# lunarring/latentblending

Measured on NVIDIA H100. Metric: transition frames/sec (1024^2 SDXL, 30 steps, 15 branches), higher is better.
Workload: dtype f16

## Files before the change

include/lb200.h:

```cpp
#ifndef LB200_H
#define LB200_H

#include <stddef.h>
#include <stdint.h>

#ifdef __cplusplus
extern "C" {
#endif

#define LB_ABI_VERSION 2

typedef struct lb_ctx lb_ctx;

int         lb_abi_version(void);
const char* lb_last_error(void);
int lb_ctx_create(int device, lb_ctx** out);
int lb_ctx_destroy(lb_ctx* ctx);
int lb_ctx_sm_count(lb_ctx* ctx);

size_t lb_slerp_workspace_bytes(int64_t rows, int64_t n);
int lb_slerp_rows(lb_ctx* ctx, const void* p0_dev, const void* p1_dev, void* out_dev,
                  int64_t rows, int64_t n, int64_t stride0, int64_t stride1, int64_t stride_out,
                  int dtype, double fract, const double* fract_rows_dev,
                  void* workspace_dev, void* stream);
// ... 17 lines not shown
    int32_t taps;
    const void* w; int64_t w_ld;
    int32_t N;
    const void* bias;
    const void* bias2; int64_t bias2_ld;
    const void* res; int64_t res_ld;
    void* out; int64_t out_ld;
    int32_t mode;
    const void* ln_stats; int32_t ln_parts;
    const void* ln_csum; const void* ln_bias;
    float ln_eps;
    void* stats_out; int32_t stats_parts;
} lb_gemm_desc;
#define LB_GEMM_STATIC_W 0x100
#define LB_GEMM_RELU 0x200
#define LB_GEMM_GEGLU256 0x400
int lb_gemm(lb_ctx* ctx, const lb_gemm_desc* desc, void* stream);
int lb_gemm_stats_parts(lb_ctx* ctx, const lb_gemm_desc* desc);

typedef struct lb_attn_desc {
    const void* q; int64_t q_ld; int32_t q_col0;
    const void* k; int64_t k_ld; int32_t k_col0;
    const void* v; int64_t v_ld; int32_t v_col0;
    void* out; int64_t out_ld;
    int32_t B, heads, Sq, Skv, head_dim;
    float scale;
} lb_attn_desc;
int lb_attention(lb_ctx* ctx, const lb_attn_desc* desc, void* stream);

size_t lb_groupnorm_workspace_bytes(lb_ctx* ctx, int B, int HW, int groups);
int lb_groupnorm(lb_ctx* ctx, const void* x, int64_t ld, int B, int HW, int C, int groups,
// ... 82 lines not shown
```

latentblending_b200/_cabi.py:

```python
import ctypes
import os
import threading

_HERE = os.path.dirname(os.path.abspath(__file__))
LIB_PATH = os.path.join(_HERE, "liblb200.so")

c_void_p, c_int, c_int64, c_float, c_double, c_size_t = (
    ctypes.c_void_p, ctypes.c_int, ctypes.c_int64, ctypes.c_float, ctypes.c_double, ctypes.c_size_t)

class GemmDesc(ctypes.Structure):
    _fields_ = [("a0", c_void_p), ("a0_ld", c_int64), ("a0_c", ctypes.c_int32),
                ("a1", c_void_p), ("a1_ld", c_int64), ("a1_c", ctypes.c_int32),
                ("B", ctypes.c_int32), ("H", ctypes.c_int32), ("W", ctypes.c_int32),
                ("taps", ctypes.c_int32),
                ("w", c_void_p), ("w_ld", c_int64),
                ("N", ctypes.c_int32),
                ("bias", c_void_p),
                ("bias2", c_void_p), ("bias2_ld", c_int64),
                ("res", c_void_p), ("res_ld", c_int64),
                ("out", c_void_p), ("out_ld", c_int64),
                ("mode", ctypes.c_int32),
                ("ln_stats", c_void_p), ("ln_parts", ctypes.c_int32),
                ("ln_csum", c_void_p), ("ln_bias", c_void_p), ("ln_eps", c_float),
                ("stats_out", c_void_p), ("stats_parts", ctypes.c_int32)]
# ... 47 lines not shown
    _fields_ = [("x", c_void_p), ("ld_x", c_int64), ("H", c_int32), ("W", c_int32), ("C", c_int32), ("k", c_int32),
                ("stride", c_int32), ("pad", c_int32), ("out", c_void_p), ("ld_out", c_int64), ("f", c_float * 6)]


class _OpUnion(ctypes.Union):
    _fields_ = [("gemm", GemmDesc), ("attn", AttnDesc), ("norm", _NormOp), ("embed", _EmbedOp), ("lin", _LinOp),
                ("conv", _ConvOp), ("resample", _ResampleOp), ("aux", _AuxOp), ("patch", _PatchOp)]


class Op(ctypes.Structure):
    _fields_ = [("kind", c_int32), ("reserved", c_int32), ("u", _OpUnion)]


GEMM_STATIC_W = 0x100
GEMM_RELU = 0x200
GEMM_GEGLU256 = 0x400
(OP_GEMM, OP_ATTENTION, OP_GROUPNORM, OP_LAYERNORM, OP_EMBED_INPUTS, OP_LINEAR_SMALL, OP_CONV_IN, OP_CONV_OUT,
 OP_UPSAMPLE2X, OP_IM2COL_S2, OP_LATENT_PREP, OP_SOFTMAX_ROWS, OP_POSTPROCESS_U8, OP_LPIPS_IM2COL_U8, OP_IM2COL,
 OP_MAXPOOL3S2, OP_NHWC_TO_NCHW) = range(1, 18)


SIGNATURES = {
    "lb_abi_version": (c_int, []),
    "lb_last_error": (ctypes.c_char_p, []),
    "lb_ctx_create": (c_int, [c_int, ctypes.POINTER(c_void_p)]),
    "lb_ctx_destroy": (c_int, [c_void_p]),
    "lb_ctx_sm_count": (c_int, [c_void_p]),
    "lb_slerp_workspace_bytes": (c_size_t, [c_int64, c_int64]),
    "lb_slerp_rows": (c_int, [c_void_p, c_void_p, c_void_p, c_void_p, c_int64, c_int64, c_int64, c_int64, c_int64,
                              c_int, c_double, c_void_p, c_void_p, c_void_p]),
    "lb_lerp": (c_int, [c_void_p, c_void_p, c_void_p, c_void_p, c_int64, c_int, c_double, c_void_p]),
# ... 98 lines not shown
```

latentblending_b200/csrc/gemm_sm90.cu:

```cuda
#include "gemm_sm90.cuh"
#include <stdlib.h>

#include "sm90.cuh"

using namespace sm90;

namespace {

constexpr int kBM = 128;
constexpr int kBK = 64;
constexpr int kEpiParts = 4;
constexpr int kThreadsGemm = 384;
constexpr int kABytes = kBM * kBK * 2;

template <int BN> struct Cfg {
    static constexpr int b_bytes = BN * kBK * 2;
    static constexpr int stage_bytes = kABytes + b_bytes;
    static constexpr int deep = (BN <= 64) ? 8 : (BN <= 128) ? 7 : (BN <= 160) ? 6 : 4;
    static constexpr int smem_bytes(int nst) { return nst * stage_bytes + 1024  + 256 ; }
};

__device__ __forceinline__ float gelu_erf(float x) {
    const float z = fabsf(x) * 0.70710678118654752440f;
    const float t = __frcp_rn(fmaf(0.3275911f, z, 1.0f));
    float poly = fmaf(1.061405429f, t, -1.453152027f);
    poly = fmaf(poly, t, 1.421413741f);
    poly = fmaf(poly, t, -0.284496736f);
    poly = fmaf(poly, t, 0.254829592f);
    const float erfc_abs = poly * t * exp2f(-1.4426950408889634f * z * z);
    const float one_plus_erf = x >= 0.f ? 2.0f - erfc_abs : erfc_abs;
    return 0.5f * x * one_plus_erf;
}

__device__ __forceinline__ float2 ld_h2(const __half* p) {
    return __half22float2(__ldg(reinterpret_cast<const __half2*>(p)));
}
__device__ __forceinline__ float2 ld_f2(const float* p) { return __ldg(reinterpret_cast<const float2*>(p)); }

__device__ __forceinline__ void ln_row_stats(const GemmParams& p, long long row, bool ok, float& mu, float& rstd) {
    mu = 0.f;
    rstd = 1.f;
    if (!ok) return;
    float s = 0.f, q = 0.f;
    const float4* st = reinterpret_cast<const float4*>(p.ln_stats + row * p.ln_parts);
    const int pairs = p.ln_parts >> 1;
    for (int base = 0; base < pairs; base += 8) {
        float4 v[8];
#pragma unroll
        for (int i = 0; i < 8; ++i) v[i] = (base + i < pairs) ? __ldcg(st + base + i) : make_float4(0.f, 0.f, 0.f, 0.f);
#pragma unroll
        for (int i = 0; i < 8; ++i) {
            s += v[i].x;
            q += v[i].y;
            s += v[i].z;
            q += v[i].w;
        }
    }
    mu = s * p.ln_inv_k;
    double var = (double)q * (double)p.ln_inv_k - (double)mu * (double)mu;
    if (var < 0.0) var = 0.0;
    rstd = rsqrtf((float)var + p.ln_eps);
}

template <int BN>
__global__ void __launch_bounds__(kThreadsGemm, 1) gemm_tc_kernel(const __grid_constant__ GemmParams p) {
    using C = Cfg<BN>;
    pdl_launch_dependents();
    extern __shared__ uint8_t smem_raw[];
    const uint32_t raw_addr = smem_u32(smem_raw);
    uint8_t* smem = smem_raw + ((1024u - (raw_addr & 1023u)) & 1023u);
    uint8_t* smem_a = smem;
    const int nst = p.stages;
    uint8_t* smem_b = smem + nst * kABytes;
    uint64_t* bars = reinterpret_cast<uint64_t*>(smem + nst * C::stage_bytes);
    uint64_t* full = bars;
    uint64_t* empty = bars + nst;

    const int warp = uniform_warp_idx(), lane = threadIdx.x & 31;
    const int wg = warp >> 2;

    if (warp == 0 && lane == 0) {
        tma_prefetch_desc(&p.tmA[0]);
        tma_prefetch_desc(&p.tmA[1]);
        tma_prefetch_desc(&p.tmB);
        for (int s = 0; s < nst; ++s) {
            mbar_init(&full[s], 1);
            mbar_init(&empty[s], 2);
        }
        fence_mbar_init();
    }
    __syncthreads();

    const int m_groups = p.tiles_m;
    const int num_tiles = m_groups * p.tiles_n;
    const int tile0 = (int)blockIdx.x;
    const int tile_step = (int)gridDim.x;

    int early_kb = 0;
    if (p.static_w && tile0 < num_tiles) early_kb = p.total_kb < nst ? p.total_kb : nst;
    if (warp == 0 && early_kb > 0) {
        if (elect_one()) {
            const int n_tile = tile0 / m_groups;
            for (int kb = 0; kb < early_kb; ++kb) {
// ... 30 lines not shown
                            tma_load_2d(smem_b + stage * C::b_bytes, &p.tmB, &full[stage], kb_global * kBK, n_tile * BN);
                        }
                    }
                    __syncwarp();
                    if (++stage == nst) { stage = 0; phase ^= 1; }
                }
            }
        }
        return;
    }

    reg_alloc<232>();
    const int cw = wg - 1;
    const bool wg_leader = (threadIdx.x & 127) == 0;
    const int quad = lane & 3;
    int rr[2], ww[2], hh[2], bb[2];
#pragma unroll
    for (int i = 0; i < 2; ++i) {
        rr[i] = cw * 64 + (warp & 3) * 16 + (lane >> 2) + 8 * i;
        ww[i] = rr[i] % p.tw;
        hh[i] = (rr[i] / p.tw) % p.th;
        bb[i] = rr[i] / (p.tw * p.th);
    }
    float acc[BN / 2];
    int stage = 0;
    uint32_t phase = 0;
    for (int tile = tile0; tile < num_tiles; tile += tile_step) {
        const int m_tile = tile % m_groups, n_tile = tile / m_groups;
        bool row_ok[2];
        long long row[2];
        int bidx[2];
        float ln_mu[2] = {0.f, 0.f}, ln_rstd[2] = {1.f, 1.f};
#pragma unroll
        for (int i = 0; i < 2; ++i) {
            const int x = (m_tile % p.tiles_x) * p.tw + ww[i];
            const int y = ((m_tile / p.tiles_x) % p.tiles_y) * p.th + hh[i];
            const int b = (m_tile / (p.tiles_x * p.tiles_y)) * p.tb + bb[i];
            row_ok[i] = (x < p.W) && (y < p.H) && (b < p.B);
            row[i] = ((long long)b * p.H + y) * p.W + x;
            bidx[i] = b;
            if (p.ln_stats) ln_row_stats(p, row[i], row_ok[i], ln_mu[i], ln_rstd[i]);
        }
        int prev_stage = -1;
        for (int kb = 0; kb < p.total_kb; ++kb) {
            mbar_wait(&full[stage], phase, p.err_flag, 3);
            const uint32_t a_addr = smem_u32(smem_a + stage * kABytes) + cw * (64 * 128);
            const uint32_t b_addr = smem_u32(smem_b + stage * C::b_bytes);
            fence_regs(acc);
            wgmma_fence();
#pragma unroll
            for (int k = 0; k < kBK / 16; ++k)
                WgmmaSS<BN>::template mma<0>(acc, make_smem_desc_sw128(a_addr + k * 32, 16, 1024),
                                             make_smem_desc_sw128(b_addr + k * 32, 16, 1024), (kb | k) != 0);
            wgmma_commit();
            wgmma_wait<1>();
            fence_regs(acc);
            if (prev_stage >= 0 && wg_leader) mbar_arrive(&empty[prev_stage]);
            prev_stage = stage;
            if (++stage == nst) { stage = 0; phase ^= 1; }
        }
        wgmma_wait<0>();
        fence_regs(acc);
        if (prev_stage >= 0 && wg_leader) mbar_arrive(&empty[prev_stage]);

        if (p.mode == 0) {
            const int n_base = n_tile * BN + 2 * quad;
#pragma unroll
            for (int i = 0; i < 2; ++i) {
                float st_sum = 0.f, st_sq = 0.f;
                if (row_ok[i]) {
                    const __half* res_row = p.res ? p.res + row[i] * p.ldr : nullptr;
                    __half* out_row = p.out + row[i] * p.ldo;
#pragma unroll
                    for (int j = 0; j < BN / 8; ++j) {
                        const int n = n_base + 8 * j;
                        if (n < p.N) {
                            float v0 = acc[4 * j + 2 * i], v1 = acc[4 * j + 2 * i + 1];
                            if (p.ln_stats) {
                                const float2 c = ld_f2(p.ln_csum + n), t = ld_f2(p.ln_bias + n);
                                v0 = fmaf(ln_rstd[i], v0 - ln_mu[i] * c.x, t.x);
                                v1 = fmaf(ln_rstd[i], v1 - ln_mu[i] * c.y, t.y);
                            } else if (p.bias) {
                                const float2 t = ld_h2(p.bias + n);
                                v0 += t.x;
                                v1 += t.y;
                            }
                            if (p.bias2) {
                                const float2 t = ld_h2(p.bias2 + (long long)bidx[i] * p.bias2_ld + n);
                                v0 += t.x;
                                v1 += t.y;
                            }
                            if (res_row) {
                                const float2 t = __half22float2(*reinterpret_cast<const __half2*>(res_row + n));
                                v0 += t.x;
                                v1 += t.y;
                            }
                            if (p.relu) {
                                v0 = fmaxf(v0, 0.f);
                                v1 = fmaxf(v1, 0.f);
                            }
                            const __half2 o = __floats2half2_rn(v0, v1);
                            *reinterpret_cast<__half2*>(out_row + n) = o;
                            if (p.stats_out) {
                                const float2 f = __half22float2(o);
                                st_sum += f.x + f.y;
                                st_sq = fmaf(f.x, f.x, fmaf(f.y, f.y, st_sq));
                            }
                        }
                    }
                    if (p.stats_out)
                        p.stats_out[row[i] * (kEpiParts * p.tiles_n) + kEpiParts * n_tile + quad] =
                            make_float2(st_sum, st_sq);
                }
            }
        } else {
            constexpr int HN = BN / 2;
            const int o_base = n_tile * HN + 2 * quad;
            const int a_base = n_tile * BN + 2 * quad;
#pragma unroll
            for (int i = 0; i < 2; ++i) {
                if (!row_ok[i]) continue;
                __half* out_row = p.out + row[i] * p.ldo;
#pragma unroll
                for (int j = 0; j < HN / 8; ++j) {
                    float v[2] = {acc[4 * j + 2 * i], acc[4 * j + 2 * i + 1]};
                    float g[2] = {acc[4 * (j + HN / 8) + 2 * i], acc[4 * (j + HN / 8) + 2 * i + 1]};
                    float2 bv = make_float2(0.f, 0.f), bg = make_float2(0.f, 0.f);
                    if (p.ln_stats) {
                        const float2 cv = ld_f2(p.ln_csum + a_base + 8 * j), cg = ld_f2(p.ln_csum + a_base + HN + 8 * j);
                        bv = ld_f2(p.ln_bias + a_base + 8 * j);
                        bg = ld_f2(p.ln_bias + a_base + HN + 8 * j);
                        v[0] = ln_rstd[i] * (v[0] - ln_mu[i] * cv.x);
                        v[1] = ln_rstd[i] * (v[1] - ln_mu[i] * cv.y);
                        g[0] = ln_rstd[i] * (g[0] - ln_mu[i] * cg.x);
                        g[1] = ln_rstd[i] * (g[1] - ln_mu[i] * cg.y);
                    } else if (p.bias) {
                        bv = ld_h2(p.bias + a_base + 8 * j);
                        bg = ld_h2(p.bias + a_base + HN + 8 * j);
                    }
                    const float r0 = lb_round_h(v[0] + bv.x) * lb_round_h(gelu_erf(lb_round_h(g[0] + bg.x)));
                    const float r1 = lb_round_h(v[1] + bv.y) * lb_round_h(gelu_erf(lb_round_h(g[1] + bg.y)));
                    *reinterpret_cast<__half2*>(out_row + o_base + 8 * j) = __floats2half2_rn(r0, r1);
                }
            }
        }
    }
}


typedef CUresult (*EncodeTiledFn)(CUtensorMap*, CUtensorMapDataType, cuuint32_t, void*, const cuuint64_t*,
                                  const cuuint64_t*, const cuuint32_t*, const cuuint32_t*, CUtensorMapInterleave,
                                  CUtensorMapSwizzle, CUtensorMapL2promotion, CUtensorMapFloatOOBfill);

int get_encode(lb_ctx* ctx, EncodeTiledFn* fn) {
    if (!ctx->tmap_encode) {
        void* f = nullptr;
        cudaDriverEntryPointQueryResult qres;
        LB_CHECK_CUDA(cudaGetDriverEntryPoint("cuTensorMapEncodeTiled", &f, cudaEnableDefault, &qres));
        LB_REQUIRE(f != nullptr && qres == cudaDriverEntryPointSuccess, "cuTensorMapEncodeTiled not available");
// ... 32 lines not shown
    cuuint32_t estr[2] = {1, 1};
    CUresult r = enc(m, CU_TENSOR_MAP_DATA_TYPE_FLOAT16, 2, const_cast<void*>(base), dims, strides, box, estr,
                     CU_TENSOR_MAP_INTERLEAVE_NONE, CU_TENSOR_MAP_SWIZZLE_128B, CU_TENSOR_MAP_L2_PROMOTION_L2_256B,
                     CU_TENSOR_MAP_FLOAT_OOB_FILL_NONE);
    LB_REQUIRE(r == CUDA_SUCCESS, "cuTensorMapEncodeTiled(weight K=%lld N=%d bn=%d) failed: %d", (long long)K, N, bn,
               (int)r);
    return 0;
}

bool is_pow2(int v) { return v > 0 && (v & (v - 1)) == 0; }

template <int BN> int launch_bn(const GemmPlan& plan, cudaStream_t st) {
    static bool attr_set = false;
    if (!attr_set) {
        LB_CHECK_CUDA(cudaFuncSetAttribute(gemm_tc_kernel<BN>, cudaFuncAttributeMaxDynamicSharedMemorySize,
                                           Cfg<BN>::smem_bytes(Cfg<BN>::deep)));
        attr_set = true;
    }
    LB_CHECK_CUDA(lb_launch_pdl(gemm_tc_kernel<BN>, dim3((unsigned)plan.grid), dim3(kThreadsGemm),
                                (size_t)Cfg<BN>::smem_bytes(plan.p.stages), st, plan.p));
    return 0;
}

}

int gemm_plan_build(lb_ctx* ctx, const GemmDesc& d, GemmPlan* plan) {
    LB_REQUIRE(ctx && plan, "gemm: null ctx/plan");
    LB_REQUIRE(d.a0 && d.w && d.out, "gemm: null a0/w/out");
    LB_REQUIRE(d.B >= 1 && d.H >= 1 && d.W >= 1 && d.N >= 8, "gemm: bad shape B=%d H=%d W=%d N=%d", d.B, d.H, d.W, d.N);
    LB_REQUIRE(d.taps == 1 || d.taps == 9, "gemm: taps must be 1 or 9");
    LB_REQUIRE(d.a0_c % kBK == 0 && d.a0_c > 0, "gemm: a0 channels (%d) must be a multiple of 64", d.a0_c);
    LB_REQUIRE(d.a1 == nullptr || (d.a1_c % kBK == 0 && d.a1_c > 0), "gemm: a1 channels must be a multiple of 64");
    LB_REQUIRE(d.N % 8 == 0, "gemm: N (%d) must be a multiple of 8", d.N);
    LB_REQUIRE(d.out_ld % 8 == 0 && lb_aligned16(d.out), "gemm: out must be 16B aligned with ld %% 8 == 0");
    LB_REQUIRE(!d.res || (d.res_ld % 8 == 0 && lb_aligned16(d.res)), "gemm: residual alignment");
// ... 10 lines not shown
        th = kBM / tw;
        if (th > d.H) {
            LB_REQUIRE(is_pow2(d.H), "gemm: H (%d) must be a power of two when H*W < 128", d.H);
            th = d.H;
        }
        tb = kBM / (tw * th);
    }
    p.tw = tw; p.th = th; p.tb = tb;
    p.W = d.W; p.H = d.H; p.B = d.B;
    p.tiles_x = (int)lb_ceil_div(d.W, tw);
    p.tiles_y = (int)lb_ceil_div(d.H, th);
    const int tiles_b = (int)lb_ceil_div(d.B, tb);
    p.tiles_m = p.tiles_x * p.tiles_y * tiles_b;
    int bn;
    if ((d.mode & 0xff) == 1) {
        bn = (d.mode & LB_GEMM_GEGLU256) ? 256 : 128;
        LB_REQUIRE(d.N % bn == 0, "gemm: GEGLU needs N %% %d == 0 (got %d)", bn, d.N);
    } else if (d.N % 256 == 0 && (int64_t)p.tiles_m * (d.N / 256) >= 2 * ctx->sm_count) bn = 256;
    else if (d.N % 160 == 0) bn = 160;
    else if (d.N % 128 == 0) bn = 128;
    else if (d.N <= 64) bn = 64;
    else bn = 128;
    plan->bn = bn;
    p.tiles_n = (int)lb_ceil_div(d.N, bn);
    p.N = d.N;
    p.mode = d.mode & 0xff;
    p.static_w = (d.mode & LB_GEMM_STATIC_W) ? 1 : 0;
    int ns = 0, total = 0;
    if (d.taps == 9) {
        for (int ky = 0; ky < 3; ++ky)
            for (int kx = 0; kx < 3; ++kx) {
                p.seg_map[ns] = 0; p.seg_dy[ns] = ky - 1; p.seg_dx[ns] = kx - 1; p.seg_kb[ns] = d.a0_c / kBK;
                total += p.seg_kb[ns++];
            }
    } else {
        p.seg_map[ns] = 0; p.seg_dy[ns] = 0; p.seg_dx[ns] = 0; p.seg_kb[ns] = d.a0_c / kBK;
        total += p.seg_kb[ns++];
    }
    if (d.a1) {
        p.seg_map[ns] = 1; p.seg_dy[ns] = 0; p.seg_dx[ns] = 0; p.seg_kb[ns] = d.a1_c / kBK;
// ... 30 lines not shown
        p.ln_csum = static_cast<const float*>(d.ln_csum);
        p.ln_bias = static_cast<const float*>(d.ln_bias);
        p.ln_inv_k = 1.0f / (float)d.a0_c;
        p.ln_eps = d.ln_eps;
    }
    if (d.stats_out) {
        LB_REQUIRE(p.mode == 0, "gemm: stats_out needs the linear epilogue");
        LB_REQUIRE(d.stats_parts == kEpiParts * p.tiles_n, "gemm: stats_parts must be %d * ceil(N / %d) = %d (got %d)",
                   kEpiParts, bn, kEpiParts * p.tiles_n, d.stats_parts);
        p.stats_out = static_cast<float2*>(d.stats_out);
    }
    {
        const int tiles = p.tiles_m * p.tiles_n;
        plan->grid = tiles < ctx->sm_count ? tiles : ctx->sm_count;
    }
    p.stages = (bn <= 64) ? 8 : (bn <= 128) ? 7 : (bn <= 160) ? 6 : 4;
    return 0;
}

int gemm_plan_launch(const GemmPlan& plan, cudaStream_t st) {
    switch (plan.bn) {
        case 64: return launch_bn<64>(plan, st);
        case 128: return launch_bn<128>(plan, st);
        case 160: return launch_bn<160>(plan, st);
        case 256: return launch_bn<256>(plan, st);
    }
    lb_set_error("gemm: unsupported N tile %d", plan.bn);
    return 2;
}

extern "C" int lb_gemm_stats_parts(lb_ctx* ctx, const lb_gemm_desc* desc) {
// ... 16 lines not shown
```

latentblending_b200/csrc/gemm_sm90.cuh:

```cuda
#pragma once
#include "common.cuh"

struct GemmDesc {
    const void* a0; int64_t a0_ld; int32_t a0_c;
    const void* a1; int64_t a1_ld; int32_t a1_c;
    int32_t B, H, W;
    int32_t taps;
    const void* w; int64_t w_ld;
    int32_t N;
    const void* bias;
    const void* bias2; int64_t bias2_ld;
    const void* res; int64_t res_ld;
    void* out; int64_t out_ld;
    int32_t mode;
    const void* ln_stats; int32_t ln_parts;
    const void* ln_csum; const void* ln_bias; float ln_eps;
    void* stats_out; int32_t stats_parts;
};

constexpr int kGemmMaxSegs = 12;

struct alignas(64) GemmParams {
    CUtensorMap tmA[2];
    CUtensorMap tmB;
    int num_segs;
    int seg_map[kGemmMaxSegs], seg_dy[kGemmMaxSegs], seg_dx[kGemmMaxSegs], seg_kb[kGemmMaxSegs];
    int total_kb;
    int W, H, B;
    int tw, th, tb;
    int tiles_x, tiles_y, tiles_m, tiles_n;
    int N;
    int mode;
    int stages;
    int static_w;
    __half* out; long long ldo;
    const __half* bias;
    const __half* bias2; long long bias2_ld;
    const __half* res; long long ldr;
    int* err_flag;
    int relu;
    const float2* ln_stats; int ln_parts; float ln_inv_k, ln_eps;
    const float* ln_csum; const float* ln_bias;
    float2* stats_out;
};

struct GemmPlan {
    GemmParams p;
    int bn;
// ... 7 lines not shown
```

latentblending_b200/unet.py:

```python
import ctypes
import os
from dataclasses import dataclass
from typing import Tuple

import torch

from . import _cabi
from ._cabi import (GEMM_GEGLU256, GEMM_RELU, GEMM_STATIC_W, OP_ATTENTION, OP_CONV_IN, OP_CONV_OUT, OP_EMBED_INPUTS, OP_GEMM,
                    OP_GROUPNORM, OP_IM2COL, OP_IM2COL_S2, OP_LATENT_PREP, OP_LAYERNORM, OP_LINEAR_SMALL,
                    OP_LPIPS_IM2COL_U8, OP_MAXPOOL3S2, OP_NHWC_TO_NCHW, OP_POSTPROCESS_U8, OP_SOFTMAX_ROWS, OP_UPSAMPLE2X, Op, check, ctx,
                    stream_ptr)


@dataclass
class UNetConfig:
    in_channels: int = 4
    out_channels: int = 4
    block_out_channels: Tuple[int, ...] = (320, 640, 1280)
    layers_per_block: int = 2
    transformer_layers: Tuple[int, ...] = (0, 2, 10)
    head_dim: int = 64
    cross_attention_dim: int = 2048
    addition_time_embed_dim: int = 256
    pooled_dim: int = 1280
# ... 229 lines not shown
    wf = (w.float() * gamma.float()[None, :]).half().contiguous()
    csum = wf.float().sum(dim=1).contiguous()
    lnb = w.float() @ beta.float()
    if bias is not None:
        lnb = lnb + bias.float()
    return wf, csum, lnb.contiguous()


def _geglu_perm(inner, device, half=64):
    idx = torch.arange(inner, device=device).view(-1, half)
    return torch.stack([idx, idx + inner], dim=1).reshape(-1)


class PackedUNet:

    def __init__(self, cfg: UNetConfig, state_dict, device, fold_ln=True, geglu_tile=128):
        self.cfg = cfg
        self.device = torch.device(device)
        self.fold_ln = fold_ln
        self.geglu_tile = geglu_tile
        sd = state_dict
        dev = self.device

        def g(name):
            return sd[name].detach().to(device=dev, dtype=torch.float16).contiguous()

        def conv3(name):
            w = g(name + ".weight")
            return w.permute(0, 2, 3, 1).reshape(w.shape[0], -1).contiguous()

        self.g = g
        self.w = {}
        W = self.w
        W["conv_in.w"] = g("conv_in.weight").permute(2, 3, 1, 0).contiguous()
        W["conv_in.b"] = g("conv_in.bias")
# ... 31 lines not shown
            W[a + ".norm.g"], W[a + ".norm.b"] = g(a + ".norm.weight"), g(a + ".norm.bias")
            W[a + ".proj_in.w"], W[a + ".proj_in.b"] = g(a + ".proj_in.weight"), g(a + ".proj_in.bias")
            W[a + ".proj_out.w"], W[a + ".proj_out.b"] = g(a + ".proj_out.weight"), g(a + ".proj_out.bias")
            depth = 0
            while f"{a}.transformer_blocks.{depth}.norm1.weight" in sd:
                t = f"{a}.transformer_blocks.{depth}"
                for n in ("norm1", "norm2", "norm3"):
                    W[f"{t}.{n}.g"], W[f"{t}.{n}.b"] = g(f"{t}.{n}.weight"), g(f"{t}.{n}.bias")
                wqkv = torch.cat([g(t + ".attn1.to_q.weight"), g(t + ".attn1.to_k.weight"),
                                  g(t + ".attn1.to_v.weight")], 0).contiguous()
                W[t + ".attn1.out.w"], W[t + ".attn1.out.b"] = g(t + ".attn1.to_out.0.weight"), g(t + ".attn1.to_out.0.bias")
                wq = g(t + ".attn2.to_q.weight")
                W[t + ".attn2.kv.w"] = torch.cat([g(t + ".attn2.to_k.weight"), g(t + ".attn2.to_v.weight")], 0).contiguous()
                W[t + ".attn2.out.w"], W[t + ".attn2.out.b"] = g(t + ".attn2.to_out.0.weight"), g(t + ".attn2.to_out.0.bias")
                pw, pb = g(t + ".ff.net.0.proj.weight"), g(t + ".ff.net.0.proj.bias")
                perm = _geglu_perm(pw.shape[0] // 2, dev, half=geglu_tile // 2)
                if fold_ln:
                    for key, w_, b_, nrm, pm in ((".attn1.qkv", wqkv, None, "norm1", None), (".attn2.q", wq, None, "norm2", None),
                                                 (".ff.in", pw, pb, "norm3", perm)):
                        wf, cs, lb = _fold_layernorm(w_, b_, W[f"{t}.{nrm}.g"], W[f"{t}.{nrm}.b"])
                        if pm is not None:
                            wf, cs, lb = wf[pm].contiguous(), cs[pm].contiguous(), lb[pm].contiguous()
                        W[t + key + ".w"], W[t + key + ".csum"], W[t + key + ".lnb"] = wf, cs, lb
                else:
                    W[t + ".attn1.qkv.w"], W[t + ".attn2.q.w"] = wqkv, wq
                    W[t + ".ff.in.w"], W[t + ".ff.in.b"] = pw[perm].contiguous(), pb[perm].contiguous()
                W[t + ".ff.out.w"], W[t + ".ff.out.b"] = g(t + ".ff.net.2.weight"), g(t + ".ff.net.2.bias")
                depth += 1
            W[a + ".depth"] = depth
        for k in sd:
            if k.endswith("samplers.0.conv.weight"):
# ... 2 lines not shown

    def nbytes(self):
        return sum(t.numel() * t.element_size() for t in self.w.values() if torch.is_tensor(t))


class UNetB200:

    def __init__(self, cfg: UNetConfig, state_dict, device="cuda:0", fold_ln=None):
        import os
        self.cfg = cfg
        self.device = torch.device(device)
        self.dev_index = self.device.index or 0
        if fold_ln is None:
            fold_ln = os.environ.get("LB_LN_FOLD") is not None
        self.fold_ln = fold_ln
        tile = int(os.environ.get("LB_GEGLU_TILE", "256"))
        widths = [c for c, d in zip(cfg.block_out_channels, cfg.transformer_layers) if d]
        if tile == 256 and any((8 * c) % 256 for c in widths):
            tile = 128
        self.geglu_tile = tile
        self.packed = PackedUNet(cfg, state_dict, self.device, fold_ln=fold_ln, geglu_tile=tile)
        self._plans = {}

    def plan(self, B, H, W, tag=None, x_in=None):
        key = (B, H, W) if tag is None else (B, H, W, tag)
        if key not in self._plans:
            self._plans[key] = _Lowering(self, B, H, W, x_in=x_in)
        return self._plans[key]

    @torch.no_grad()
    def forward(self, x, t, encoder_hidden_states, text_embeds, time_ids, ctx_changed=True):
        B, _, H, W = x.shape
        pl = self.plan(B, H, W)
        pl.x_in.copy_(x)
        pl.text.copy_(text_embeds)
        pl.tids.copy_(time_ids)
# ... 92 lines not shown
            M = rows_at(level)
            n1 = scratch("n1", M, cin)
            P.groupnorm(x, B, h_ * w_, cin, groups, Wt[rname + ".norm1.g"], Wt[rname + ".norm1.b"], 1e-5, 1, n1, self.ws)
            h1 = scratch("h1", M, cout)
            P.gemm(n1, Wt[rname + ".conv1.w"], cout, B, h_, w_, h1, taps=9, bias=Wt[rname + ".conv1.b"], bias2=tslice(rname))
            n2 = scratch("n2", M, cout)
            P.groupnorm(h1, B, h_ * w_, cout, groups, Wt[rname + ".norm2.g"], Wt[rname + ".norm2.b"], 1e-5, 1, n2, self.ws)
            if Wt.get(rname + ".has_shortcut"):
                P.gemm(n2, Wt[rname + ".conv2.w"], cout, B, h_, w_, out, taps=9, a1=x, a1_c=cin, bias=Wt[rname + ".conv2.b"])
            else:
                P.gemm(n2, Wt[rname + ".conv2.w"], cout, B, h_, w_, out, taps=9, bias=Wt[rname + ".conv2.b"], res=x)

        kv_cache = {}

        fold = net.fold_ln
        geglu_mode = 1 | (GEMM_GEGLU256 if net.geglu_tile == 256 else 0)
        f32 = dict(dtype=torch.float32, device=dev)

        def transformer(aname, x, C, level, out):
            h_, w_ = res_hw[level]
            S = h_ * w_
            M = rows_at(level)
            heads = C // cfg.head_dim
            tn = scratch("tn", M, C)
            P.groupnorm(x, B, S, C, groups, Wt[aname + ".norm.g"], Wt[aname + ".norm.b"], 1e-6, 0, tn, self.ws)
            hs = scratch("hs", M, C)
            if not fold:
                P.gemm(tn, Wt[aname + ".proj_in.w"], C, 1, 1, M, hs, bias=Wt[aname + ".proj_in.b"])
                stats = None
            else:
                parts = P.gemm_stats_parts(tn, Wt[aname + ".proj_in.w"], C, 1, 1, M, hs)
# ... 116 lines not shown
```

Before: 1.397.

## Ping-pong consumer warpgroups across tiles and drop the GEGLU 256 tile path

For tile widths of 160 or less, the two consumer warpgroups now each take whole 128-row tiles and alternate through the mainloop using turn barriers. This lets one group's epilogue overlap the other's MMAs. Stage counts become compile-time constants, the GEGLU path is fixed to a 128-wide tile, and epilogue loads are batched ahead of the arithmetic. The 256-wide tile is now chosen only for large-K GEMMs. The changes risk extra register pressure from the double accumulators, and GEGLU GEMMs lose the wider tile they used by default before.

```diff
diff --git a/include/lb200.h b/include/lb200.h
--- a/include/lb200.h
+++ b/include/lb200.h
@@ -55,7 +55,6 @@
 } lb_gemm_desc;
 #define LB_GEMM_STATIC_W 0x100
 #define LB_GEMM_RELU 0x200
-#define LB_GEMM_GEGLU256 0x400
 int lb_gemm(lb_ctx* ctx, const lb_gemm_desc* desc, void* stream);
 int lb_gemm_stats_parts(lb_ctx* ctx, const lb_gemm_desc* desc);
 
diff --git a/latentblending_b200/_cabi.py b/latentblending_b200/_cabi.py
--- a/latentblending_b200/_cabi.py
+++ b/latentblending_b200/_cabi.py
@@ -85,7 +85,6 @@
 
 GEMM_STATIC_W = 0x100
 GEMM_RELU = 0x200
-GEMM_GEGLU256 = 0x400
 (OP_GEMM, OP_ATTENTION, OP_GROUPNORM, OP_LAYERNORM, OP_EMBED_INPUTS, OP_LINEAR_SMALL, OP_CONV_IN, OP_CONV_OUT,
  OP_UPSAMPLE2X, OP_IM2COL_S2, OP_LATENT_PREP, OP_SOFTMAX_ROWS, OP_POSTPROCESS_U8, OP_LPIPS_IM2COL_U8, OP_IM2COL,
  OP_MAXPOOL3S2, OP_NHWC_TO_NCHW) = range(1, 18)
diff --git a/latentblending_b200/csrc/gemm_sm90.cu b/latentblending_b200/csrc/gemm_sm90.cu
--- a/latentblending_b200/csrc/gemm_sm90.cu
+++ b/latentblending_b200/csrc/gemm_sm90.cu
@@ -12,12 +12,15 @@
 constexpr int kEpiParts = 4;
 constexpr int kThreadsGemm = 384;
 constexpr int kABytes = kBM * kBK * 2;
+constexpr int kGegluBN = 128;
 
 template <int BN> struct Cfg {
     static constexpr int b_bytes = BN * kBK * 2;
     static constexpr int stage_bytes = kABytes + b_bytes;
-    static constexpr int deep = (BN <= 64) ? 8 : (BN <= 128) ? 7 : (BN <= 160) ? 6 : 4;
-    static constexpr int smem_bytes(int nst) { return nst * stage_bytes + 1024  + 256 ; }
+    static constexpr int stages = (BN <= 64) ? 8 : (BN <= 128) ? 7 : (BN <= 160) ? 6 : 4;
+    static constexpr bool coop = BN > 160;
+    static constexpr int smem_bytes = stages * stage_bytes + 1024  + 256 ;
+    static_assert(smem_bytes <= 227 * 1024, "smem ring does not fit");
 };
 
 __device__ __forceinline__ float gelu_erf(float x) {
@@ -32,10 +35,8 @@
     return 0.5f * x * one_plus_erf;
 }
 
-__device__ __forceinline__ float2 ld_h2(const __half* p) {
-    return __half22float2(__ldg(reinterpret_cast<const __half2*>(p)));
-}
 __device__ __forceinline__ float2 ld_f2(const float* p) { return __ldg(reinterpret_cast<const float2*>(p)); }
+__device__ __forceinline__ __half2 ld_h2(const __half* p) { return __ldg(reinterpret_cast<const __half2*>(p)); }
 
 __device__ __forceinline__ void ln_row_stats(const GemmParams& p, long long row, bool ok, float& mu, float& rstd) {
     mu = 0.f;
@@ -62,19 +63,172 @@
     rstd = rsqrtf((float)var + p.ln_eps);
 }
 
+struct EpiRow {
+    long long row;
+    int bidx;
+    bool ok;
+    float ln_mu, ln_rstd;
+};
+
+template <int BN>
+__device__ __forceinline__ void epilogue_linear(const GemmParams& p, const float (&acc)[BN / 2], const EpiRow (&r)[2],
+                                                int n_tile, int quad) {
+    constexpr int G = BN / 8;
+    constexpr int CH = G > 10 ? G / 2 : G;
+    static_assert(G % CH == 0, "load batches must tile the row");
+    const int n_base = n_tile * BN + 2 * quad;
+#pragma unroll
+    for (int i = 0; i < 2; ++i) {
+        if (!r[i].ok) continue;
+        float st_sum = 0.f, st_sq = 0.f;
+        const __half* res_row = p.res ? p.res + r[i].row * p.ldr : nullptr;
+        const __half* b2_row = p.bias2 ? p.bias2 + (long long)r[i].bidx * p.bias2_ld : nullptr;
+        __half* out_row = p.out + r[i].row * p.ldo;
+#pragma unroll
+        for (int c0 = 0; c0 < G; c0 += CH) {
+            float v[CH][2];
+#pragma unroll
+            for (int g = 0; g < CH; ++g) {
+                v[g][0] = acc[4 * (c0 + g) + 2 * i];
+                v[g][1] = acc[4 * (c0 + g) + 2 * i + 1];
+            }
+            if (p.ln_stats) {
+                constexpr int CL = CH > 8 ? CH / 2 : CH;
+#pragma unroll
+                for (int l0 = 0; l0 < CH; l0 += CL) {
+                    float2 c[CL], t[CL];
+#pragma unroll
+                    for (int g = 0; g < CL; ++g) {
+                        const int n = n_base + 8 * (c0 + l0 + g);
+                        c[g] = n < p.N ? ld_f2(p.ln_csum + n) : make_float2(0.f, 0.f);
+                        t[g] = n < p.N ? ld_f2(p.ln_bias + n) : make_float2(0.f, 0.f);
+                    }
+#pragma unroll
+                    for (int g = 0; g < CL; ++g) {
+                        v[l0 + g][0] = fmaf(r[i].ln_rstd, v[l0 + g][0] - r[i].ln_mu * c[g].x, t[g].x);
+                        v[l0 + g][1] = fmaf(r[i].ln_rstd, v[l0 + g][1] - r[i].ln_mu * c[g].y, t[g].y);
+                    }
+                }
+            } else {
+                const __half2 z = __float2half2_rn(0.f);
+                __half2 hb[CH], hb2[CH], hr[CH];
+#pragma unroll
+                for (int g = 0; g < CH; ++g) {
+                    const int n = n_base + 8 * (c0 + g);
+                    const bool in = n < p.N;
+                    hb[g] = (p.bias && in) ? ld_h2(p.bias + n) : z;
+                    hb2[g] = (b2_row && in) ? ld_h2(b2_row + n) : z;
+                    hr[g] = (res_row && in) ? *reinterpret_cast<const __half2*>(res_row + n) : z;
+                }
+#pragma unroll
+                for (int g = 0; g < CH; ++g) {
+                    if (p.bias) {
+                        const float2 t = __half22float2(hb[g]);
+                        v[g][0] += t.x;
+                        v[g][1] += t.y;
+                    }
+                    if (b2_row) {
+                        const float2 t = __half22float2(hb2[g]);
+                        v[g][0] += t.x;
+                        v[g][1] += t.y;
+                    }
+                    if (res_row) {
+                        const float2 t = __half22float2(hr[g]);
+                        v[g][0] += t.x;
+                        v[g][1] += t.y;
+                    }
+                }
+            }
+#pragma unroll
+            for (int g = 0; g < CH; ++g) {
+                const int n = n_base + 8 * (c0 + g);
+                if (n < p.N) {
+                    float v0 = v[g][0], v1 = v[g][1];
+                    if (p.relu) {
+                        v0 = fmaxf(v0, 0.f);
+                        v1 = fmaxf(v1, 0.f);
+                    }
+                    const __half2 o = __floats2half2_rn(v0, v1);
+                    *reinterpret_cast<__half2*>(out_row + n) = o;
+                    if (p.stats_out) {
+                        const float2 f = __half22float2(o);
+                        st_sum += f.x + f.y;
+                        st_sq = fmaf(f.x, f.x, fmaf(f.y, f.y, st_sq));
+                    }
+                }
+            }
+        }
+        if (p.stats_out)
+            p.stats_out[r[i].row * (kEpiParts * p.tiles_n) + kEpiParts * n_tile + quad] = make_float2(st_sum, st_sq);
+    }
+}
+
+template <int BN>
+__device__ __forceinline__ void epilogue_geglu(const GemmParams& p, const float (&acc)[BN / 2], const EpiRow (&r)[2],
+                                               int n_tile, int quad) {
+    constexpr int HN = BN / 2;
+    constexpr int G = HN / 8;
+    const int o_base = n_tile * HN + 2 * quad;
+    const int a_base = n_tile * BN + 2 * quad;
+#pragma unroll
+    for (int i = 0; i < 2; ++i) {
+        if (!r[i].ok) continue;
+        __half* out_row = p.out + r[i].row * p.ldo;
+        float2 bv[G], bg[G];
+        if (p.ln_stats) {
+            float2 cv[G], cg[G];
+#pragma unroll
+            for (int j = 0; j < G; ++j) {
+                cv[j] = ld_f2(p.ln_csum + a_base + 8 * j);
+                cg[j] = ld_f2(p.ln_csum + a_base + HN + 8 * j);
+                bv[j] = ld_f2(p.ln_bias + a_base + 8 * j);
+                bg[j] = ld_f2(p.ln_bias + a_base + HN + 8 * j);
+            }
+#pragma unroll
+            for (int j = 0; j < G; ++j) {
+                float v[2] = {acc[4 * j + 2 * i], acc[4 * j + 2 * i + 1]};
+                float g[2] = {acc[4 * (j + G) + 2 * i], acc[4 * (j + G) + 2 * i + 1]};
+                v[0] = r[i].ln_rstd * (v[0] - r[i].ln_mu * cv[j].x);
+                v[1] = r[i].ln_rstd * (v[1] - r[i].ln_mu * cv[j].y);
+                g[0] = r[i].ln_rstd * (g[0] - r[i].ln_mu * cg[j].x);
+                g[1] = r[i].ln_rstd * (g[1] - r[i].ln_mu * cg[j].y);
+                const float r0 = lb_round_h(v[0] + bv[j].x) * lb_round_h(gelu_erf(lb_round_h(g[0] + bg[j].x)));
+                const float r1 = lb_round_h(v[1] + bv[j].y) * lb_round_h(gelu_erf(lb_round_h(g[1] + bg[j].y)));
+                *reinterpret_cast<__half2*>(out_row + o_base + 8 * j) = __floats2half2_rn(r0, r1);
+            }
+        } else {
+#pragma unroll
+            for (int j = 0; j < G; ++j) {
+                bv[j] = p.bias ? __half22float2(ld_h2(p.bias + a_base + 8 * j)) : make_float2(0.f, 0.f);
+                bg[j] = p.bias ? __half22float2(ld_h2(p.bias + a_base + HN + 8 * j)) : make_float2(0.f, 0.f);
+            }
+#pragma unroll
+            for (int j = 0; j < G; ++j) {
+                const float r0 = lb_round_h(acc[4 * j + 2 * i] + bv[j].x) *
+                                 lb_round_h(gelu_erf(lb_round_h(acc[4 * (j + G) + 2 * i] + bg[j].x)));
+                const float r1 = lb_round_h(acc[4 * j + 2 * i + 1] + bv[j].y) *
+                                 lb_round_h(gelu_erf(lb_round_h(acc[4 * (j + G) + 2 * i + 1] + bg[j].y)));
+                *reinterpret_cast<__half2*>(out_row + o_base + 8 * j) = __floats2half2_rn(r0, r1);
+            }
+        }
+    }
+}
+
 template <int BN>
 __global__ void __launch_bounds__(kThreadsGemm, 1) gemm_tc_kernel(const __grid_constant__ GemmParams p) {
     using C = Cfg<BN>;
+    constexpr int nst = C::stages;
+    constexpr bool kCoop = C::coop;
     pdl_launch_dependents();
     extern __shared__ uint8_t smem_raw[];
     const uint32_t raw_addr = smem_u32(smem_raw);
     uint8_t* smem = smem_raw + ((1024u - (raw_addr & 1023u)) & 1023u);
     uint8_t* smem_a = smem;
-    const int nst = p.stages;
     uint8_t* smem_b = smem + nst * kABytes;
     uint64_t* bars = reinterpret_cast<uint64_t*>(smem + nst * C::stage_bytes);
     uint64_t* full = bars;
     uint64_t* empty = bars + nst;
+    uint64_t* turn = bars + 2 * nst;
 
     const int warp = uniform_warp_idx(), lane = threadIdx.x & 31;
     const int wg = warp >> 2;
@@ -85,8 +239,10 @@
         tma_prefetch_desc(&p.tmB);
         for (int s = 0; s < nst; ++s) {
             mbar_init(&full[s], 1);
-            mbar_init(&empty[s], 2);
-        }
+            mbar_init(&empty[s], kCoop ? 2 : 1);
+        }
+        mbar_init(&turn[0], 128);
+        mbar_init(&turn[1], 128);
         fence_mbar_init();
     }
     __syncthreads();
@@ -147,135 +303,95 @@
     const int cw = wg - 1;
     const bool wg_leader = (threadIdx.x & 127) == 0;
     const int quad = lane & 3;
-    int rr[2], ww[2], hh[2], bb[2];
-#pragma unroll
-    for (int i = 0; i < 2; ++i) {
-        rr[i] = cw * 64 + (warp & 3) * 16 + (lane >> 2) + 8 * i;
-        ww[i] = rr[i] % p.tw;
-        hh[i] = (rr[i] / p.tw) % p.th;
-        bb[i] = rr[i] / (p.tw * p.th);
-    }
-    float acc[BN / 2];
-    int stage = 0;
-    uint32_t phase = 0;
-    for (int tile = tile0; tile < num_tiles; tile += tile_step) {
+    const int my_tiles = tile0 < num_tiles ? (num_tiles - tile0 + tile_step - 1) / tile_step : 0;
+    constexpr int kHalves = kCoop ? 1 : 2;
+    float acc[kHalves][BN / 2];
+    const auto half_of = [&](int hh) { return kCoop ? cw : hh; };
+    for (int j = kCoop ? 0 : cw; j < my_tiles; j += kCoop ? 1 : 2) {
+        const int tile = tile0 + j * tile_step;
         const int m_tile = tile % m_groups, n_tile = tile / m_groups;
-        bool row_ok[2];
-        long long row[2];
-        int bidx[2];
-        float ln_mu[2] = {0.f, 0.f}, ln_rstd[2] = {1.f, 1.f};
-#pragma unroll
-        for (int i = 0; i < 2; ++i) {
-            const int x = (m_tile % p.tiles_x) * p.tw + ww[i];
-            const int y = ((m_tile / p.tiles_x) % p.tiles_y) * p.th + hh[i];
-            const int b = (m_tile / (p.tiles_x * p.tiles_y)) * p.tb + bb[i];
-            row_ok[i] = (x < p.W) && (y < p.H) && (b < p.B);
-            row[i] = ((long long)b * p.H + y) * p.W + x;
-            bidx[i] = b;
-            if (p.ln_stats) ln_row_stats(p, row[i], row_ok[i], ln_mu[i], ln_rstd[i]);
+        EpiRow er[kHalves][2];
+        const auto row_of = [&](int hh, int i) {
+            const int rr = half_of(hh) * 64 + (warp & 3) * 16 + (lane >> 2) + 8 * i;
+            const int x = (m_tile % p.tiles_x) * p.tw + rr % p.tw;
+            const int y = ((m_tile / p.tiles_x) % p.tiles_y) * p.th + (rr / p.tw) % p.th;
+            const int b = (m_tile / (p.tiles_x * p.tiles_y)) * p.tb + rr / (p.tw * p.th);
+            EpiRow& e = er[hh][i];
+            e.ok = (x < p.W) && (y < p.H) && (b < p.B);
+            e.row = ((long long)b * p.H + y) * p.W + x;
+            e.bidx = b;
+        };
+        float ln_mu[kHalves][2], ln_rstd[kHalves][2];
+#pragma unroll
+        for (int hh = 0; hh < kHalves; ++hh)
+#pragma unroll
+            for (int i = 0; i < 2; ++i) {
+                ln_mu[hh][i] = 0.f;
+                ln_rstd[hh][i] = 1.f;
+                if (p.ln_stats) {
+                    row_of(hh, i);
+                    ln_row_stats(p, er[hh][i].row, er[hh][i].ok, ln_mu[hh][i], ln_rstd[hh][i]);
+                }
+            }
+        const uint32_t it0 = (uint32_t)j * (uint32_t)p.total_kb;
+        int stage = (int)(it0 % nst);
+        uint32_t phase = (it0 / nst) & 1u;
+#pragma unroll
+        for (int hh = 0; hh < kHalves; ++hh)
+#pragma unroll
+            for (int i = 0; i < BN / 2; ++i) acc[hh][i] = 0.f;
+        if (!kCoop && j > 0) {
+            const uint32_t par = (uint32_t)((j - 1) >> 1) & 1u;
+            if (cw == 0) mbar_wait(&turn[0], par, p.err_flag, 4);
+            else mbar_wait(&turn[1], par, p.err_flag, 4);
         }
         int prev_stage = -1;
         for (int kb = 0; kb < p.total_kb; ++kb) {
             mbar_wait(&full[stage], phase, p.err_flag, 3);
-            const uint32_t a_addr = smem_u32(smem_a + stage * kABytes) + cw * (64 * 128);
+            const uint32_t a_addr = smem_u32(smem_a + stage * kABytes);
             const uint32_t b_addr = smem_u32(smem_b + stage * C::b_bytes);
-            fence_regs(acc);
+#pragma unroll
+            for (int hh = 0; hh < kHalves; ++hh) fence_regs(acc[hh]);
             wgmma_fence();
 #pragma unroll
-            for (int k = 0; k < kBK / 16; ++k)
-                WgmmaSS<BN>::template mma<0>(acc, make_smem_desc_sw128(a_addr + k * 32, 16, 1024),
-                                             make_smem_desc_sw128(b_addr + k * 32, 16, 1024), (kb | k) != 0);
+            for (int k = 0; k < kBK / 16; ++k) {
+                const uint64_t bdesc = make_smem_desc_sw128(b_addr + k * 32, 16, 1024);
+#pragma unroll
+                for (int hh = 0; hh < kHalves; ++hh)
+                    WgmmaSS<BN>::template mma<0>(acc[hh],
+                                                 make_smem_desc_sw128(a_addr + half_of(hh) * (64 * 128) + k * 32, 16,
+                                                                      1024),
+                                                 bdesc, (kb | k) != 0);
+            }
             wgmma_commit();
             wgmma_wait<1>();
-            fence_regs(acc);
+#pragma unroll
+            for (int hh = 0; hh < kHalves; ++hh) fence_regs(acc[hh]);
             if (prev_stage >= 0 && wg_leader) mbar_arrive(&empty[prev_stage]);
             prev_stage = stage;
             if (++stage == nst) { stage = 0; phase ^= 1; }
         }
+        if (!kCoop && j + 1 < my_tiles) {
+            if (cw == 0) mbar_arrive(&turn[1]);
+            else mbar_arrive(&turn[0]);
+        }
         wgmma_wait<0>();
-        fence_regs(acc);
+#pragma unroll
+        for (int hh = 0; hh < kHalves; ++hh) fence_regs(acc[hh]);
         if (prev_stage >= 0 && wg_leader) mbar_arrive(&empty[prev_stage]);
-
-        if (p.mode == 0) {
-            const int n_base = n_tile * BN + 2 * quad;
+#pragma unroll
+        for (int hh = 0; hh < kHalves; ++hh)
 #pragma unroll
             for (int i = 0; i < 2; ++i) {
-                float st_sum = 0.f, st_sq = 0.f;
-                if (row_ok[i]) {
-                    const __half* res_row = p.res ? p.res + row[i] * p.ldr : nullptr;
-                    __half* out_row = p.out + row[i] * p.ldo;
-#pragma unroll
-                    for (int j = 0; j < BN / 8; ++j) {
-                        const int n = n_base + 8 * j;
-                        if (n < p.N) {
-                            float v0 = acc[4 * j + 2 * i], v1 = acc[4 * j + 2 * i + 1];
-                            if (p.ln_stats) {
-                                const float2 c = ld_f2(p.ln_csum + n), t = ld_f2(p.ln_bias + n);
-                                v0 = fmaf(ln_rstd[i], v0 - ln_mu[i] * c.x, t.x);
-                                v1 = fmaf(ln_rstd[i], v1 - ln_mu[i] * c.y, t.y);
-                            } else if (p.bias) {
-                                const float2 t = ld_h2(p.bias + n);
-                                v0 += t.x;
-                                v1 += t.y;
-                            }
-                            if (p.bias2) {
-                                const float2 t = ld_h2(p.bias2 + (long long)bidx[i] * p.bias2_ld + n);
-                                v0 += t.x;
-                                v1 += t.y;
-                            }
-                            if (res_row) {
-                                const float2 t = __half22float2(*reinterpret_cast<const __half2*>(res_row + n));
-                                v0 += t.x;
-                                v1 += t.y;
-                            }
-                            if (p.relu) {
-                                v0 = fmaxf(v0, 0.f);
-                                v1 = fmaxf(v1, 0.f);
-                            }
-                            const __half2 o = __floats2half2_rn(v0, v1);
-                            *reinterpret_cast<__half2*>(out_row + n) = o;
-                            if (p.stats_out) {
-                                const float2 f = __half22float2(o);
-                                st_sum += f.x + f.y;
-                                st_sq = fmaf(f.x, f.x, fmaf(f.y, f.y, st_sq));
-                            }
-                        }
-                    }
-                    if (p.stats_out)
-                        p.stats_out[row[i] * (kEpiParts * p.tiles_n) + kEpiParts * n_tile + quad] =
-                            make_float2(st_sum, st_sq);
-                }
-            }
-        } else {
-            constexpr int HN = BN / 2;
-            const int o_base = n_tile * HN + 2 * quad;
-            const int a_base = n_tile * BN + 2 * quad;
-#pragma unroll
-            for (int i = 0; i < 2; ++i) {
-                if (!row_ok[i]) continue;
-                __half* out_row = p.out + row[i] * p.ldo;
-#pragma unroll
-                for (int j = 0; j < HN / 8; ++j) {
-                    float v[2] = {acc[4 * j + 2 * i], acc[4 * j + 2 * i + 1]};
-                    float g[2] = {acc[4 * (j + HN / 8) + 2 * i], acc[4 * (j + HN / 8) + 2 * i + 1]};
-                    float2 bv = make_float2(0.f, 0.f), bg = make_float2(0.f, 0.f);
-                    if (p.ln_stats) {
-                        const float2 cv = ld_f2(p.ln_csum + a_base + 8 * j), cg = ld_f2(p.ln_csum + a_base + HN + 8 * j);
-                        bv = ld_f2(p.ln_bias + a_base + 8 * j);
-                        bg = ld_f2(p.ln_bias + a_base + HN + 8 * j);
-                        v[0] = ln_rstd[i] * (v[0] - ln_mu[i] * cv.x);
-                        v[1] = ln_rstd[i] * (v[1] - ln_mu[i] * cv.y);
-                        g[0] = ln_rstd[i] * (g[0] - ln_mu[i] * cg.x);
-                        g[1] = ln_rstd[i] * (g[1] - ln_mu[i] * cg.y);
-                    } else if (p.bias) {
-                        bv = ld_h2(p.bias + a_base + 8 * j);
-                        bg = ld_h2(p.bias + a_base + HN + 8 * j);
-                    }
-                    const float r0 = lb_round_h(v[0] + bv.x) * lb_round_h(gelu_erf(lb_round_h(g[0] + bg.x)));
-                    const float r1 = lb_round_h(v[1] + bv.y) * lb_round_h(gelu_erf(lb_round_h(g[1] + bg.y)));
-                    *reinterpret_cast<__half2*>(out_row + o_base + 8 * j) = __floats2half2_rn(r0, r1);
-                }
-            }
+                row_of(hh, i);
+                er[hh][i].ln_mu = ln_mu[hh][i];
+                er[hh][i].ln_rstd = ln_rstd[hh][i];
+            }
+
+#pragma unroll
+        for (int hh = 0; hh < kHalves; ++hh) {
+            if (p.mode == 0) epilogue_linear<BN>(p, acc[hh], er[hh], n_tile, quad);
+            else if constexpr (BN == kGegluBN) epilogue_geglu<BN>(p, acc[hh], er[hh], n_tile, quad);
         }
     }
 }
@@ -338,11 +454,11 @@
     static bool attr_set = false;
     if (!attr_set) {
         LB_CHECK_CUDA(cudaFuncSetAttribute(gemm_tc_kernel<BN>, cudaFuncAttributeMaxDynamicSharedMemorySize,
-                                           Cfg<BN>::smem_bytes(Cfg<BN>::deep)));
+                                           Cfg<BN>::smem_bytes));
         attr_set = true;
     }
     LB_CHECK_CUDA(lb_launch_pdl(gemm_tc_kernel<BN>, dim3((unsigned)plan.grid), dim3(kThreadsGemm),
-                                (size_t)Cfg<BN>::smem_bytes(plan.p.stages), st, plan.p));
+                                (size_t)Cfg<BN>::smem_bytes, st, plan.p));
     return 0;
 }
 
@@ -383,16 +499,20 @@
     p.tiles_m = p.tiles_x * p.tiles_y * tiles_b;
     int bn;
     if ((d.mode & 0xff) == 1) {
-        bn = (d.mode & LB_GEMM_GEGLU256) ? 256 : 128;
+        bn = kGegluBN;
         LB_REQUIRE(d.N % bn == 0, "gemm: GEGLU needs N %% %d == 0 (got %d)", bn, d.N);
-    } else if (d.N % 256 == 0 && (int64_t)p.tiles_m * (d.N / 256) >= 2 * ctx->sm_count) bn = 256;
-    else if (d.N % 160 == 0) bn = 160;
+    } else if (d.N % 256 == 0 && d.N >= 512 && (int64_t)(d.taps * d.a0_c + (d.a1 ? d.a1_c : 0)) >= 4096 &&
+               (int64_t)p.tiles_m * (d.N / 256) >= 2 * ctx->sm_count) {
+        bn = 256;
+    } else if (d.N % 160 == 0) bn = 160;
     else if (d.N % 128 == 0) bn = 128;
     else if (d.N <= 64) bn = 64;
     else bn = 128;
     plan->bn = bn;
     p.tiles_n = (int)lb_ceil_div(d.N, bn);
     p.N = d.N;
+    LB_REQUIRE((d.mode & ~(0xff | LB_GEMM_STATIC_W | LB_GEMM_RELU)) == 0, "gemm: unknown mode flags 0x%x", d.mode);
+    LB_REQUIRE((d.mode & 0xff) <= 1, "gemm: unknown epilogue mode %d", d.mode & 0xff);
     p.mode = d.mode & 0xff;
     p.static_w = (d.mode & LB_GEMM_STATIC_W) ? 1 : 0;
     int ns = 0, total = 0;
@@ -453,7 +573,6 @@
         const int tiles = p.tiles_m * p.tiles_n;
         plan->grid = tiles < ctx->sm_count ? tiles : ctx->sm_count;
     }
-    p.stages = (bn <= 64) ? 8 : (bn <= 128) ? 7 : (bn <= 160) ? 6 : 4;
     return 0;
 }
 
diff --git a/latentblending_b200/csrc/gemm_sm90.cuh b/latentblending_b200/csrc/gemm_sm90.cuh
--- a/latentblending_b200/csrc/gemm_sm90.cuh
+++ b/latentblending_b200/csrc/gemm_sm90.cuh
@@ -31,7 +31,6 @@
     int tiles_x, tiles_y, tiles_m, tiles_n;
     int N;
     int mode;
-    int stages;
     int static_w;
     __half* out; long long ldo;
     const __half* bias;
diff --git a/latentblending_b200/unet.py b/latentblending_b200/unet.py
--- a/latentblending_b200/unet.py
+++ b/latentblending_b200/unet.py
@@ -6,7 +6,7 @@
 import torch
 
 from . import _cabi
-from ._cabi import (GEMM_GEGLU256, GEMM_RELU, GEMM_STATIC_W, OP_ATTENTION, OP_CONV_IN, OP_CONV_OUT, OP_EMBED_INPUTS, OP_GEMM,
+from ._cabi import (GEMM_RELU, GEMM_STATIC_W, OP_ATTENTION, OP_CONV_IN, OP_CONV_OUT, OP_EMBED_INPUTS, OP_GEMM,
                     OP_GROUPNORM, OP_IM2COL, OP_IM2COL_S2, OP_LATENT_PREP, OP_LAYERNORM, OP_LINEAR_SMALL,
                     OP_LPIPS_IM2COL_U8, OP_MAXPOOL3S2, OP_NHWC_TO_NCHW, OP_POSTPROCESS_U8, OP_SOFTMAX_ROWS, OP_UPSAMPLE2X, Op, check, ctx,
                     stream_ptr)
@@ -267,11 +267,10 @@
 
 class PackedUNet:
 
-    def __init__(self, cfg: UNetConfig, state_dict, device, fold_ln=True, geglu_tile=128):
+    def __init__(self, cfg: UNetConfig, state_dict, device, fold_ln=True):
         self.cfg = cfg
         self.device = torch.device(device)
         self.fold_ln = fold_ln
-        self.geglu_tile = geglu_tile
         sd = state_dict
         dev = self.device
 
@@ -333,7 +332,7 @@
                 W[t + ".attn2.kv.w"] = torch.cat([g(t + ".attn2.to_k.weight"), g(t + ".attn2.to_v.weight")], 0).contiguous()
                 W[t + ".attn2.out.w"], W[t + ".attn2.out.b"] = g(t + ".attn2.to_out.0.weight"), g(t + ".attn2.to_out.0.bias")
                 pw, pb = g(t + ".ff.net.0.proj.weight"), g(t + ".ff.net.0.proj.bias")
-                perm = _geglu_perm(pw.shape[0] // 2, dev, half=geglu_tile // 2)
+                perm = _geglu_perm(pw.shape[0] // 2, dev)
                 if fold_ln:
                     for key, w_, b_, nrm, pm in ((".attn1.qkv", wqkv, None, "norm1", None), (".attn2.q", wq, None, "norm2", None),
                                                  (".ff.in", pw, pb, "norm3", perm)):
@@ -366,12 +365,7 @@
         if fold_ln is None:
             fold_ln = os.environ.get("LB_LN_FOLD") is not None
         self.fold_ln = fold_ln
-        tile = int(os.environ.get("LB_GEGLU_TILE", "256"))
-        widths = [c for c, d in zip(cfg.block_out_channels, cfg.transformer_layers) if d]
-        if tile == 256 and any((8 * c) % 256 for c in widths):
-            tile = 128
-        self.geglu_tile = tile
-        self.packed = PackedUNet(cfg, state_dict, self.device, fold_ln=fold_ln, geglu_tile=tile)
+        self.packed = PackedUNet(cfg, state_dict, self.device, fold_ln=fold_ln)
         self._plans = {}
 
     def plan(self, B, H, W, tag=None, x_in=None):
@@ -494,7 +488,7 @@
         kv_cache = {}
 
         fold = net.fold_ln
-        geglu_mode = 1 | (GEMM_GEGLU256 if net.geglu_tile == 256 else 0)
+        geglu_mode = 1
         f32 = dict(dtype=torch.float32, device=dev)
 
         def transformer(aname, x, C, level, out):
```

Result: faster. 1.567, median of 6 (+12.2%).
